# jesselasse/MARL-DMFB

Hardware: AMD Instinct MI355X
Metric: env-steps/sec (whole node), 10x10 DMFB 4-droplet fov9 (higher is better)
Workload: dtype int8 env state/obs + f64 rewards; fp32 Q-net; 1 GPU; DMFB 10x10, drop_num=4, fov=9, 4096 parallel envs per GPU (BASELINE configs[1]); parallelism=dp1: chips sharded per rank, one flat RCCL all-reduce per learn

## Files before the change

### __graft_entry__.py

```python
import os
import subprocess
import sys

ROOT = os.path.dirname(os.path.abspath(__file__))
if ROOT not in sys.path:
    sys.path.insert(0, ROOT)


def build():
    jobs = str(max(1, min(8, os.cpu_count() or 1)))
    env = dict(os.environ, PYTORCH_ROCM_ARCH='gfx950')
    subprocess.check_call(['make', '-C', os.path.join(ROOT, 'marl_dmfb_amd', 'csrc'), '-j', jobs, '-s'], env=env)
    subprocess.check_call(['make', '-C', os.path.join(ROOT, 'oracle'), '-s'], env=env)
    import marl_dmfb_amd
    from marl_dmfb_amd import _lib
    lib = _lib.dmfb_vec()
    for name in _lib.DMFB_VEC_SYMBOLS:
        getattr(lib, name)
    lib = _lib.meda_vec()
    for name in _lib.MEDA_VEC_SYMBOLS:
        getattr(lib, name)
    lib = _lib.crnn_ops()
    for name in ('crnn_conv9_forward', 'crnn_front9_forward', 'crnn_front19_forward', 'crnn_front_padded_cols', 'crnn_conv9_backward', 'crnn_conv19_backward', 'crnn_front9_forward_live', 'gru_seq_forward', 'gru_seq_backward', 'gru_seq_forward_packed', 'gru_seq_backward_packed'):
        getattr(lib, name)
    lib = _lib.crnn_fov()
    for name in _lib.SIGNATURES['crnn_fov']:
        getattr(lib, name)
    lib = _lib.rollout_ops()
    for name in ('rollout_select_actions', 'rollout_post_step', 'rollout_gru_head_select_stream', 'rollout_stream_step'):
        getattr(lib, name)
    lib = _lib.vdn_ops()
    for name in ('vdn_td_forward', 'vdn_td_backward', 'vdn_td_forward_packed', 'vdn_td_backward_packed', 'vdn_gather_units', 'vdn_clip_adam_step'):
        getattr(lib, name)
    lib = _lib.qmix_ops()
    for name in _lib.SIGNATURES['qmix_ops']:
        getattr(lib, name)
    lib = _lib.route_plan()
    for name in _lib.SIGNATURES['route_plan']:
        getattr(lib, name)


def smoke():
    import numpy as np
    import torch
    from marl_dmfb_amd.env.dmfb import VecDMFB
    from oracle.dmfb_oracle import DmfbOracle

    assert torch.cuda.is_available(), 'smoke() needs the GPU'
    cfg = dict(width=10, length=10, n_agents=4, fov=9)
    E, seed = 256, 1234
    env = VecDMFB(n_envs=E, seed=seed, device='cuda:0', **cfg)
    ora = DmfbOracle(n_envs=E, seed=seed, **cfg)
    env.reset()
    ora.reset()
    rng = np.random.default_rng(0)
    for t in range(50):
        a = rng.integers(0, 5, (E, 4)).astype(np.int32)
        obs, r, d, info = env.step(torch.as_tensor(a, device='cuda:0'), autoreset=True)
        ro, do, co, so = ora.step(a)
        term = do.all(axis=1)
        if term.any():
            ora.reset(mask=term.astype(np.uint8))
        assert np.array_equal(r.cpu().numpy().view(np.int64), ro.view(np.int64)), 'rewards differ at step %d' % t
        assert np.array_equal(d.cpu().numpy(), do), 'dones differ at step %d' % t
        assert np.array_equal(info['constraints'].cpu().numpy(), co)
# ... 26 lines not shown
```

### marl_dmfb_amd/_lib.py

```python
import ctypes as C
import os

_HERE = os.path.dirname(os.path.abspath(__file__))
LIB_DIR = os.path.join(_HERE, 'lib')
_CACHE = {}
_FILE = {'rollout_route': 'rollout_ops'}


class HipLibraryMissing(RuntimeError):
    pass


def load(name):
    if name in _CACHE:
        return _CACHE[name]
    stem = _FILE.get(name, name)
    path = os.path.join(LIB_DIR, 'lib%s%s.so' % (stem, os.environ.get('MARL_DMFB_VARIANT_' + stem.upper(), '')))
    if not os.path.exists(path):
        raise HipLibraryMissing(
            '%s not found: build the HIP extension first (python -c "import __graft_entry__ as g; g.build()" '
            'or make -C marl_dmfb_amd/csrc). There is no CPU fallback.' % path)
    import torch
    lib = C.CDLL(path)
    _CACHE[name] = lib
    return lib


class DmfbVecConfig(C.Structure):
    _fields_ = [('width', C.c_int32), ('length', C.c_int32), ('n_agents', C.c_int32), ('n_blocks', C.c_int32),
                ('fov', C.c_int32), ('stall', C.c_int32), ('b_degrade', C.c_int32), ('with_maps', C.c_int32),
                ('per_degrade', C.c_double), ('n_envs', C.c_int32), ('env_id0', C.c_uint32), ('seed', C.c_uint64),
                ('device', C.c_int32)]


class DmfbVecStepOut(C.Structure):
    _fields_ = [('d_rewards', C.c_void_p), ('d_dones', C.c_void_p), ('d_constraints', C.c_void_p),
                ('d_success', C.c_void_p), ('d_obs', C.c_void_p), ('d_team_reward', C.c_void_p),
                ('d_terminated', C.c_void_p), ('d_obs_terminal', C.c_void_p)]

# ... 130 lines not shown
        'rollout_select_actions': [vp, i32, i32, i32, vp, i32, u64, vp, vp, vp, vp, vp, i32, i32, vp],
        'rollout_gru_head_select': [vp, vp, vp, vp, vp, vp, vp, i32, i32, i32, i32, vp, i32, u64, vp, vp, vp, vp, vp, i32, i32, vp, vp],
        'rollout_gru_head_select_live': [vp, vp, vp, vp, vp, vp, vp, i32, i32, i32, i32, vp, i32, u64, vp, vp, vp, vp, vp, i32, i32, vp, vp,
                                         vp, vp],
        'rollout_compact_alive': [i32, vp, vp, vp, vp],
        'rollout_post_step': [i32, i32, i32, vp, vp, vp, vp, i32, vp, vp, vp, vp, vp, vp, vp, vp, vp, f32, f32, vp, vp, vp, i32, vp, vp,
                              vp],
        'rollout_gru_head_select_stream': [vp, vp, vp, vp, vp, vp, vp, i32, i32, i32, i32, vp, i32, u64, vp, vp, vp, vp, vp, i32, vp, vp,
                                           vp],
        'rollout_stream_step': [i32, i32, i32, i32, i32, i32, vp, vp, vp, vp, vp, vp, i32, vp, C.POINTER(RolloutStage),
                                C.POINTER(RolloutRing), i32, vp, vp, vp, f32, f32, vp, vp],
        'rollout_last_hip_error': ([], i32),
    },
    'rollout_route': {
        'rollout_route_select': [i32, i32, i32, i32, vp, vp, vp, i32, vp, vp, vp, vp, vp, vp],
        'rollout_last_hip_error': ([], i32),
    },
    'route_plan': {
        'route_plan_dmfb': [i32, i32, i32, i32, i32, vp, vp, vp, vp, vp, vp, vp, vp, vp, vp, vp],
        'route_plan_max_dim': ([], i32),
        'route_plan_lds_bytes': ([i32, i32, i32], i32),
        'route_plan_last_hip_error': ([], i32),
    },
    'vdn_ops': {
        'vdn_td_forward': [vp, vp, vp, vp, vp, vp, vp, i32, i32, i32, i32, i32, f32, vp, vp, vp, vp],
        'vdn_td_backward': [vp, vp, vp, vp, i32, i32, i32, i32, i32, vp, vp],
        'vdn_td_forward_packed': [vp, vp, vp, i32, vp, vp, vp, vp, vp, i32, i32, f32, vp, vp, vp, vp],
        'vdn_td_backward_packed': [vp, vp, vp, i32, vp, vp, i32, i32, vp, vp],
        'vdn_gather_units': [vp, i32, vp, i32, i32, i32, vp, vp],
        'vdn_clip_adam_step': [i32, C.POINTER(vp), C.POINTER(vp), C.POINTER(vp), C.POINTER(vp), C.POINTER(i64), f32, f64, f64, f64,
                               f64, f64, f64, vp, vp, vp, vp],
        'vdn_last_hip_error': ([], i32),
    },
    'qmix_ops': {
        'qmix_mix_td_forward': [vp, vp, vp, vp, vp, vp, vp, i32, i32, i32, i32, i32, vp, i32, i32, vp, i32, i32, i32, i32,
                                C.POINTER(QmixMixer), C.POINTER(QmixMixer), f32, vp, vp, vp, vp],
        'qmix_mix_td_backward': [vp, vp, vp, vp, i32, i32, i32, i32, i32, vp, i32, i32, i32, i32, C.POINTER(QmixMixer), vp, vp, vp,
                                 vp, vp, vp],
        'qmix_last_hip_error': ([], i32),
    },
}

DMFB_VEC_SYMBOLS = list(SIGNATURES['dmfb_vec'])
MEDA_VEC_SYMBOLS = list(SIGNATURES['meda_vec'])

ENV_ERRORS = {
    'dmfb_vec': {
        -1: (ValueError, 'bad argument'),
        -2: (RuntimeError, 'Fov is too large'),
        -3: (TypeError, 'Too many droplets for DMFB'),
        -4: (AssertionError, 'width >= 5 and length >= 5'),
        -5: (AssertionError, 'n_agents > 0'),
        -6: (NotImplementedError, 'configuration outside the build limits (include/dmfb_vec.h)'),
        -7: (TypeError, 'action is illegal'),
        -8: (RuntimeError, 'env was created without health/usage/degrade maps (pass with_maps=True)'),
    },
    'meda_vec': {
        -1: (ValueError, 'bad argument'),
        -3: (RuntimeError, 'Too many droplets in the MEDA array'),
        -4: (AssertionError, 'w > 0 and l > 0'),
        -5: (AssertionError, 'n_agents > 0'),
        -6: (NotImplementedError, 'configuration outside the build limits (include/meda_vec.h)'),
        -8: (RuntimeError, 'env was created without health/usage/degrade maps (pass with_maps=True)'),
    },
    'route_plan': {
        -1: (ValueError, 'bad argument'),
# ... 57 lines not shown

def dmfb_vec():
    return _library('dmfb_vec')


def meda_vec():
    return _library('meda_vec')


def crnn_ops():
    return _library('crnn_ops')


def crnn_fov():
    return _library('crnn_fov')


def rollout_ops():
    return _library('rollout_ops')


def rollout_route():
    return _library('rollout_route')


def route_plan():
    return _library('route_plan')


def vdn_ops():
    return _library('vdn_ops')


def qmix_ops():
    return _library('qmix_ops')
```

### marl_dmfb_amd/csrc/crnn_ops.hip

```cpp
#include <hip/hip_runtime.h>

#include <cstdint>
#include <cstdio>
#include <cstdlib>

#include "../../include/crnn_ops.h"

#define HIP_ABI_TAG "crnn_ops"
#define HIP_ABI_ERR CRNN_ERR_HIP
#include "hip_abi.h"
#include "crnn_mfma.h"
#include "crnn_mfma19.h"
#include "crnn_bwd19.h"

namespace {

constexpr int kBlock = 512;
constexpr int kA1Stride = 52;
constexpr int kDz1Unit = 108;

constexpr int kLdsBudget = 158 * 1024;

template <int OD> struct GeoB {
    static constexpr int DZ2 = 28;
// ... 337 lines not shown
            const int pair = i / 9, tap = i - pair * 9, c2 = pair / OD, c1 = pair - c2 * OD;
            const int unit = c2 * (OD / 2) + (c1 >> 1), comp = 2 * tap + (c1 & 1);
            if (unit < G::NA) off[cnt++] = unit * 18 + comp;
            else
                for (int sl = 0; sl < G::XSLICES && sl < 8; ++sl) off[cnt++] = (G::NA + sl * G::NB + (unit - G::NA)) * 18 + comp;
        } else if (i < n2 + nb) {
            off[cnt++] = kBlock * 18 + (i - n2);
        } else if (i < n2 + nb + n1) {
            const int jx = i - n2 - nb, c1 = jx / 27, r = jx - c1 * 27, ky = r % 3;
            const int item = (c1 >> 1) * 9 + r / 3;
            for (int sl = 0; sl < G::RS3; ++sl) off[cnt++] = kBlock * 18 + OD + (sl * G::ITEMS3 + item) * 6 + (c1 & 1) * 3 + ky;
        } else {
            off[cnt++] = kBlock * 18 + OD + kBlock * 6 + (i - n2 - nb - n1);
        }
        for (int k = 0; k < cnt; ++k) {
            float a0 = 0.0f, a1 = 0.0f;
            int b = ty;
            for (; b + kRedY < n_part; b += 2 * kRedY) { a0 += part[(size_t)b * G::PART + off[k]]; a1 += part[(size_t)(b + kRedY) * G::PART + off[k]]; }
            if (b < n_part) a0 += part[(size_t)b * G::PART + off[k]];
            acc += a0 + a1;
        }
    }
    s_sum[ty][tx] = acc;
    __syncthreads();
    if (ty == 0 && i < n2 + nb + n1 + nb) {
        float t = 0.0f;
#pragma unroll
        for (int k = 0; k < kRedY; ++k) t += s_sum[k][tx];
        grads[i] = t;
    }
}

constexpr int kMlpBlock = 256, kMlpOut = 10, kMlpMaxIn = 18, kMlpMaxParts = 256;
__global__ __launch_bounds__(kMlpBlock) void k_mlp_bwd(const int8_t *__restrict__ obs, long obs_stride, int dir_off,
                                                       const int8_t *__restrict__ onehot, int n_actions, long rows,
                                                       const float *__restrict__ x, long x_stride, const float *__restrict__ g, long g_stride,
                                                       int col0, float *__restrict__ part) {
    __shared__ float s_red[kMlpBlock / 64][kMlpOut * (kMlpMaxIn + 1)];
    float acc[kMlpOut][kMlpMaxIn + 1];
#pragma unroll
    for (int o = 0; o < kMlpOut; ++o)
#pragma unroll
        for (int k = 0; k <= kMlpMaxIn; ++k) acc[o][k] = 0.0f;
    for (long r = (long)blockIdx.x * kMlpBlock + threadIdx.x; r < rows; r += (long)gridDim.x * kMlpBlock) {
        float v[kMlpMaxIn];
        v[0] = (float)obs[r * obs_stride + dir_off];
        v[1] = (float)obs[r * obs_stride + dir_off + 1];
#pragma unroll
        for (int k = 0; k < kMlpMaxIn - 2; ++k) v[2 + k] = k < n_actions ? (float)onehot[r * n_actions + k] : 0.0f;
#pragma unroll
        for (int o = 0; o < kMlpOut; ++o) {
            const float gz = x[r * x_stride + col0 + o] > 0.0f ? g[r * g_stride + col0 + o] : 0.0f;
#pragma unroll
            for (int k = 0; k < kMlpMaxIn; ++k) acc[o][k] = fmaf(gz, v[k], acc[o][k]);
            acc[o][kMlpMaxIn] += gz;
        }
    }
    const int lane = threadIdx.x & 63, wave = threadIdx.x >> 6;
#pragma unroll
    for (int o = 0; o < kMlpOut; ++o)
#pragma unroll
        for (int k = 0; k <= kMlpMaxIn; ++k) {
            float t = acc[o][k];
            for (int d = 32; d > 0; d >>= 1) t += __shfl_xor(t, d);
            if (lane == 0) s_red[wave][o * (kMlpMaxIn + 1) + k] = t;
        }
    __syncthreads();
    for (int i = threadIdx.x; i < kMlpOut * (kMlpMaxIn + 1); i += kMlpBlock) {
        float t = 0.0f;
#pragma unroll
        for (int w = 0; w < kMlpBlock / 64; ++w) t += s_red[w][i];
        part[(size_t)blockIdx.x * kMlpOut * (kMlpMaxIn + 1) + i] = t;
    }
}
__global__ __launch_bounds__(256) void k_mlp_bwd_reduce(const float *__restrict__ part, int n_part, int nin, float *__restrict__ dw, float *__restrict__ db) {
    const int i = threadIdx.x;
    if (i >= kMlpOut * nin + kMlpOut) return;
    const int o = i < kMlpOut * nin ? i / nin : i - kMlpOut * nin, k = i < kMlpOut * nin ? i - o * nin : kMlpMaxIn;
    float t = 0.0f;
    for (int b = 0; b < n_part; ++b) t += part[(size_t)b * kMlpOut * (kMlpMaxIn + 1) + o * (kMlpMaxIn + 1) + k];
    if (i < kMlpOut * nin) dw[i] = t;
    else db[o] = t;
}

struct LiveRows { const int32_t *chips; const int32_t *n; int rows_per_chip; };

template <int OD, int RBV>
int launch_rb(const int8_t *obs, long obs_stride, long rows, const float *w1, const float *b1, const float *w2, const float *b2,
              float *out, long out_stride, int out_cols, const int8_t *onehot, int n_actions, const float *mlp_w, const float *mlp_b, hipStream_t s,
              LiveRows live = LiveRows{nullptr, nullptr, 1}) {
    using GM = crnn_mfma::GeoM<OD, RBV>;
    const size_t lds = GM::LDS_FLOATS * sizeof(float);
    static LdsLimit lds_limit;
    if (const int rc = lds_limit.raise((const void *)crnn_mfma::k_conv9_mfma<OD, RBV>, lds)) return rc;
    const long n_blocks = (rows + GM::RB - 1) / GM::RB;
    const long resident = 256L * (long)((size_t)160 * 1024 / lds);
    const int grid = (int)(n_blocks < resident ? n_blocks : resident);
    LAUNCH((crnn_mfma::k_conv9_mfma<OD, RBV>), dim3(grid), dim3(crnn_mfma::kBlockM), lds, s, obs, obs_stride, rows, w1, b1, w2, b2,
           out, out_stride, out_cols, onehot, n_actions, mlp_w, mlp_b, live.chips, live.n, live.rows_per_chip);
    return CRNN_OK;
}

template <int OD>
int launch(const int8_t *obs, long obs_stride, long rows, const float *w1, const float *b1, const float *w2, const float *b2,
           float *out, long out_stride, int out_cols, const int8_t *onehot, int n_actions, const float *mlp_w, const float *mlp_b, hipStream_t s,
           LiveRows live = LiveRows{nullptr, nullptr, 1}) {
    return launch_rb<OD, 0>(obs, obs_stride, rows, w1, b1, w2, b2, out, out_stride, out_cols, onehot, n_actions, mlp_w, mlp_b, s, live);
}

template <int OD>
int launch19(const int8_t *obs, long obs_stride, long rows, const float *w1, const float *b1, const float *w3, const float *b3,
             float *out, long out_stride, int out_cols, const int8_t *onehot, int n_actions, const float *mlp_w, const float *mlp_b, hipStream_t s) {
    using GM = crnn_mfma19::Geo<OD>;
    const size_t lds = GM::LDS_FLOATS * sizeof(float);
    static LdsLimit lds_limit;
// ... 90 lines not shown
    const bool vec = d_mlp_w != nullptr;
    const int n_feat = od * 25 + (vec ? 10 : 0);
    if (!d_obs || !d_w1 || !d_b1 || !d_w3 || !d_b3 || !d_out || rows < 0 || obs_stride < 3 * 19 * 19 + (vec ? 2 : 0) ||
        out_stride < n_feat || n_actions < 0 || n_actions > 16 || (vec && !d_mlp_b))
        return CRNN_ERR_BAD_ARG;
    if (od != 24 && od != 32) return CRNN_ERR_UNSUPPORTED;
    if (out_cols != 0 && (out_cols < n_feat || out_cols > crnn_front_padded_cols(od) || out_cols > out_stride)) return CRNN_ERR_BAD_ARG;
    if (rows == 0) return CRNN_OK;
    if (od == 24) return launch19<24>(d_obs, obs_stride, rows, d_w1, d_b1, d_w3, d_b3, d_out, out_stride, out_cols, d_onehot, n_actions, d_mlp_w, d_mlp_b, (hipStream_t)stream);
    return launch19<32>(d_obs, obs_stride, rows, d_w1, d_b1, d_w3, d_b3, d_out, out_stride, out_cols, d_onehot, n_actions, d_mlp_w, d_mlp_b, (hipStream_t)stream);
}

int crnn_conv9_backward_parts(int od) { return od == 24 ? GeoB<24>::PART : od == 32 ? GeoB<32>::PART : CRNN_ERR_UNSUPPORTED; }

int crnn_conv9_backward(const int8_t *d_obs, int64_t obs_stride, int64_t rows, const float *d_out, int64_t out_stride,
                        const float *d_grad_out, int64_t grad_stride, const float *d_w1, const float *d_b1, const float *d_w2,
                        int od, float *d_part, int n_part, float *d_grads, void *stream) {
    if (!d_obs || !d_out || !d_grad_out || !d_w1 || !d_b1 || !d_w2 || !d_part || !d_grads || rows <= 0 || n_part < 1 || n_part > 256)
        return CRNN_ERR_BAD_ARG;
    if (od == 24) return launch_bwd<24>(d_obs, obs_stride, rows, d_out, out_stride, d_grad_out, grad_stride, d_w2, d_part, n_part, d_grads, d_w1, d_b1, (hipStream_t)stream);
    if (od == 32) return launch_bwd<32>(d_obs, obs_stride, rows, d_out, out_stride, d_grad_out, grad_stride, d_w2, d_part, n_part, d_grads, d_w1, d_b1, (hipStream_t)stream);
    return CRNN_ERR_UNSUPPORTED;
}

int crnn_mlp_backward_parts(void) { return kMlpMaxParts * kMlpOut * (kMlpMaxIn + 1); }

int crnn_mlp_backward(const int8_t *d_obs, int64_t obs_stride, int dir_offset, const int8_t *d_onehot, int n_actions, int64_t rows,
                      const float *d_out, int64_t out_stride, const float *d_grad_out, int64_t grad_stride, int col0, float *d_part,
                      float *d_grad_w, float *d_grad_b, void *stream) {
    if (!d_obs || !d_onehot || !d_out || !d_grad_out || !d_part || !d_grad_w || !d_grad_b || rows <= 0 || n_actions < 0 ||
        n_actions > kMlpMaxIn - 2 || dir_offset < 0 || obs_stride < dir_offset + 2 || col0 < 0 || out_stride < col0 + kMlpOut ||
        grad_stride < col0 + kMlpOut)
        return CRNN_ERR_BAD_ARG;
    const long want = (rows + kMlpBlock - 1) / kMlpBlock;
    const int grid = (int)(want < kMlpMaxParts ? want : kMlpMaxParts);
    HIP_TRY(launch_status([&] {
        hipLaunchKernelGGL(k_mlp_bwd, dim3(grid), dim3(kMlpBlock), 0, (hipStream_t)stream, d_obs, (long)obs_stride, dir_offset, d_onehot, n_actions,
                           (long)rows, d_out, (long)out_stride, d_grad_out, (long)grad_stride, col0, d_part);
        hipLaunchKernelGGL(k_mlp_bwd_reduce, dim3(1), dim3(256), 0, (hipStream_t)stream, d_part, grid, 2 + n_actions, d_grad_w, d_grad_b);
    }));
    return CRNN_OK;
}

int crnn_conv19_backward_parts(int od) { return od == 24 ? crnn_bwd19::GeoB19<24>::PART : od == 32 ? crnn_bwd19::GeoB19<32>::PART : CRNN_ERR_UNSUPPORTED; }

int crnn_conv19_backward(const int8_t *d_obs, int64_t obs_stride, int64_t rows, const float *d_out, int64_t out_stride,
                         const float *d_grad_out, int64_t grad_stride, const float *d_w1, const float *d_b1, const float *d_w3,
                         const float *d_b3, int od, float *d_part, int n_part, float *d_grads, void *stream) {
    if (!d_obs || !d_out || !d_grad_out || !d_w1 || !d_b1 || !d_w3 || !d_b3 || !d_part || !d_grads || rows <= 0 || n_part < 1 ||
        n_part > 256 || obs_stride < 3 * 19 * 19 || out_stride < od * 25 || grad_stride < od * 25)
        return CRNN_ERR_BAD_ARG;
    if (od == 24) return launch_bwd19<24>(d_obs, obs_stride, rows, d_out, out_stride, d_grad_out, grad_stride, d_w1, d_b1, d_w3, d_b3, d_part, n_part, d_grads, (hipStream_t)stream);
    if (od == 32) return launch_bwd19<32>(d_obs, obs_stride, rows, d_out, out_stride, d_grad_out, grad_stride, d_w1, d_b1, d_w3, d_b3, d_part, n_part, d_grads, (hipStream_t)stream);
    return CRNN_ERR_UNSUPPORTED;
}

int crnn_last_hip_error(void) { return g_last_hip; }

}
```

### marl_dmfb_amd/csrc/vdn_ops.hip

```cpp
#include <hip/hip_runtime.h>

#include <cstdint>

#include "../../include/vdn_ops.h"

#define HIP_ABI_TAG "vdn_ops"
#define HIP_ABI_ERR VDN_ERR_HIP
#include "hip_abi.h"

namespace {

__global__ __launch_bounds__(256) void k_td_forward(const float *__restrict__ qe, const float *__restrict__ qt, const int8_t *__restrict__ u,
                                                    const float *__restrict__ r, const int8_t *__restrict__ avail,
                                                    const uint8_t *__restrict__ term, const uint8_t *__restrict__ padded, int B, int T,
                                                    int Tl, int n, int A, float gamma, float *__restrict__ mtd, float *__restrict__ maskf,
                                                    int32_t *__restrict__ bad) {
    const int idx = blockIdx.x * blockDim.x + threadIdx.x;
    if (idx >= B * T) return;
    const int b = idx / T, t = idx - b * T;
    const size_t ep = (size_t)b * Tl + t;
    const size_t q0 = ((size_t)t * B + b) * n * A;
    float qe_tot = 0.0f, qt_tot = 0.0f;
    bool ok = true;
    for (int i = 0; i < n; ++i) {
        int a_taken = (int)u[ep * n + i];
        if ((unsigned)a_taken >= (unsigned)A) { ok = false; a_taken = 0; }
        qe_tot = qe_tot + qe[q0 + (size_t)i * A + a_taken];
        float m = -3.4e38f;
        for (int a = 0; a < A; ++a) {
            const float v = avail[(ep * n + i) * A + a] == 0 ? -9999999.0f : qt[q0 + (size_t)i * A + a];
            m = v > m ? v : m;
        }
        qt_tot = qt_tot + m;
    }
    const float not_term = 1.0f - (term[ep] ? 1.0f : 0.0f);
    const float target = r[ep] + (gamma * qt_tot) * not_term;
    const float mk = 1.0f - (padded[ep] ? 1.0f : 0.0f);
// ... 39 lines not shown
        }
        qt_tot = qt_tot + m;
    }
    const float not_term = 1.0f - (term[ep] ? 1.0f : 0.0f);
    const float target = r[ep] + (gamma * qt_tot) * not_term;
    const float mk = 1.0f - (padded[ep] ? 1.0f : 0.0f);
    mtd[j] = ok ? mk * (target - qe_tot) : __builtin_nanf("");
    maskf[j] = mk;
    if (!ok && bad) atomicAdd(bad, 1);
}

__global__ __launch_bounds__(256) void k_td_backward_packed(const float *__restrict__ mtd, const float *__restrict__ maskf, const int32_t *__restrict__ units,
                                                            const int8_t *__restrict__ u, const float *__restrict__ g, long rows, int n, int A,
                                                            float *__restrict__ gq) {
    const long row = (long)blockIdx.x * blockDim.x + threadIdx.x;
    if (row >= rows) return;
    const int i = (int)(row % n);
    const long j = row / n;
    const float d = -((2.0f * mtd[j]) * maskf[j]) * g[0];
    const int a_taken = (int)u[(size_t)units[j] * n + i];
    const bool bad_a = (unsigned)a_taken >= (unsigned)A;
    for (int a = 0; a < A; ++a) gq[row * A + a] = (bad_a || a == a_taken) ? d : 0.0f;
}

template <typename V>
__global__ __launch_bounds__(256) void k_gather_units(const V *__restrict__ src, int unit_v, const int32_t *__restrict__ units, int U, int shift,
                                                      int zero_below, V *__restrict__ dst) {
    const long idx = (long)blockIdx.x * blockDim.x + threadIdx.x;
    if (idx >= (long)U * unit_v) return;
    const int j = (int)(idx / unit_v), k = (int)(idx - (long)j * unit_v);
    dst[idx] = j < zero_below ? (V)0 : src[((size_t)units[j] + shift) * unit_v + k];
}

}

namespace {

struct TensorList {
    float *p[VDN_MAX_TENSORS];
    float *g[VDN_MAX_TENSORS];
    float *m[VDN_MAX_TENSORS];
    float *v[VDN_MAX_TENSORS];
    long off[VDN_MAX_TENSORS + 1];
    int n;
};

__device__ __forceinline__ void locate(const TensorList &tl, long i, int &k) {
    while (i >= tl.off[k + 1]) ++k;
}

__global__ __launch_bounds__(256) void k_sqnorm_partials(TensorList tl, float *__restrict__ partials, const float *__restrict__ grad_div) {
    __shared__ float s_w[4];
    const long total = tl.off[tl.n];
    const long per = (total + gridDim.x - 1) / gridDim.x;
    const long lo = (long)blockIdx.x * per, hi = min(total, lo + per);
    float acc = 0.0f;
    int k = 0;
    for (long i = lo + threadIdx.x; i < hi; i += 256) {
        locate(tl, i, k);
        float g = tl.g[k][i - tl.off[k]];
        if (grad_div) g = g / grad_div[0];
        acc = fmaf(g, g, acc);
    }
    for (int o = 32; o > 0; o >>= 1) acc += __shfl_xor(acc, o);
    if ((threadIdx.x & 63) == 0) s_w[threadIdx.x >> 6] = acc;
    __syncthreads();
// ... 111 lines not shown
           d_bad_actions);
    return VDN_OK;
}

int vdn_td_backward_packed(const float *d_mtd, const float *d_mask, const int32_t *d_units, int32_t n_units, const int8_t *d_u,
                           const float *d_grad_num, int32_t n_agents, int32_t n_actions, float *d_grad_q, void *stream) {
    if (!d_mtd || !d_mask || !d_units || !d_u || !d_grad_num || !d_grad_q || n_units < 0 || n_agents < 1 || n_actions < 1 || n_actions > 127)
        return VDN_ERR_BAD_ARG;
    if (n_units == 0) return VDN_OK;
    const long rows = (long)n_units * n_agents;
    LAUNCH(k_td_backward_packed, dim3((unsigned)((rows + 255) / 256)), dim3(256), 0, (hipStream_t)stream, d_mtd, d_mask, d_units,
           d_u, d_grad_num, rows, n_agents, n_actions, d_grad_q);
    return VDN_OK;
}

int vdn_gather_units(const void *d_src, int32_t unit_bytes, const int32_t *d_units, int32_t n_units, int32_t unit_shift,
                     int32_t zero_below, void *d_dst, void *stream) {
    if (!d_src || !d_units || !d_dst || unit_bytes < 1 || n_units < 0 || zero_below < 0) return VDN_ERR_BAD_ARG;
    if (n_units == 0) return VDN_OK;
    HIP_TRY(launch_status([&] {
        const bool dw = unit_bytes % 4 == 0 && ((size_t)d_src | (size_t)d_dst) % 4 == 0;
        const int uv = dw ? unit_bytes / 4 : unit_bytes;
        const long total = (long)n_units * uv;
        if (dw)
            hipLaunchKernelGGL((k_gather_units<uint32_t>), dim3((unsigned)((total + 255) / 256)), dim3(256), 0, (hipStream_t)stream,
                               (const uint32_t *)d_src, uv, d_units, n_units, unit_shift, zero_below, (uint32_t *)d_dst);
        else
            hipLaunchKernelGGL((k_gather_units<uint8_t>), dim3((unsigned)((total + 255) / 256)), dim3(256), 0, (hipStream_t)stream,
                               (const uint8_t *)d_src, uv, d_units, n_units, unit_shift, zero_below, (uint8_t *)d_dst);
    }));
    return VDN_OK;
}

int vdn_last_hip_error(void) { return g_last_hip; }

}
```

### marl_dmfb_amd/network/base_net.py

```python
import os

import torch
import torch.nn as nn
import torch.nn.functional as f


_CONV_PLAN = {5: [(True, 1)], 7: [(True, 1), (False, 1)], 9: [(True, 1), (False, 1)], 11: [(True, 1), (False, 1)],
              13: [(True, 1), (False, 1)], 19: [(True, 2), (False, 1), (False, 1)]}


class _ConvGemm(torch.autograd.Function):

    @staticmethod
    def forward(ctx, cols, weight2d, bias):
        ctx.save_for_backward(cols, weight2d)
        return torch.addmm(bias, cols, weight2d.t())

    @staticmethod
    def backward(ctx, g):
        cols, w = ctx.saved_tensors
        g = g.contiguous()
        gcols = g @ w if ctx.needs_input_grad[0] else None
        M, K = cols.shape
        C = g.shape[1]
# ... 289 lines not shown
        hs, gates, h0, w_hh = ctx.saved_tensors
        lib = _GRUSeqHip._lib()
        T, R, H = hs.shape
        grad_out = grad_out.contiguous()
        h0c, w = h0.contiguous(), w_hh.contiguous()
        d_ig = torch.empty((T, R, 3 * H), dtype=torch.float32, device=hs.device)
        d_hg = torch.empty_like(d_ig)
        d_h0 = torch.empty_like(h0c)
        bias_part = torch.empty((lib.gru_seq_row_blocks(R), 6 * H), dtype=torch.float32, device=hs.device)
        lib.gru_seq_backward(grad_out.data_ptr(), gates.data_ptr(), hs.data_ptr(), h0c.data_ptr(),
                             w.data_ptr(), T, R, H, d_ig.data_ptr(), d_hg.data_ptr(), d_h0.data_ptr(),
                             bias_part.data_ptr(), torch.cuda.current_stream(hs.device).cuda_stream)
        d_w_hh = torch.matmul(d_hg[0].t(), h0c)
        if T > 1:
            d_w_hh = d_w_hh + _wgrad_splitk(d_hg[1:].reshape((T - 1) * R, 3 * H), hs[:-1].reshape((T - 1) * R, H))
        d_b = bias_part.sum(0)
        return d_ig, d_h0, d_w_hh, d_b[:3 * H], d_b[3 * H:]


class _GRUSeqHipPacked(torch.autograd.Function):

    @staticmethod
    def _steps(step_rows):
        import ctypes as C
        return (C.c_int32 * len(step_rows))(*[int(v) for v in step_rows])

    @staticmethod
    def run_forward(igates, h0, w_hh, b_ih, b_hh, step_rows, save):
        lib = _GRUSeqHip._lib()
        Vp, G = igates.shape
        H, T, R, V = G // 3, len(step_rows), h0.shape[0], int(sum(step_rows))
        igates, h0, w_hh = igates.contiguous(), h0.contiguous(), w_hh.contiguous()
        hs = torch.empty((Vp, H), dtype=torch.float32, device=igates.device)
        hs[V:].zero_()
        gates = torch.empty((Vp, 4 * H), dtype=torch.float32, device=igates.device) if save else None
        lib.gru_seq_forward_packed(igates.data_ptr(), h0.data_ptr(), w_hh.data_ptr(), b_ih.data_ptr(),
                                   b_hh.data_ptr(), T, R, H, _GRUSeqHipPacked._steps(step_rows), hs.data_ptr(),
                                   gates.data_ptr() if save else None,
                                   torch.cuda.current_stream(igates.device).cuda_stream)
        return hs, gates

    @staticmethod
    def forward(ctx, igates, h0, w_hh, b_ih, b_hh, step_rows):
        hs, gates = _GRUSeqHipPacked.run_forward(igates.detach(), h0.detach(), w_hh.detach(), b_ih.detach(), b_hh.detach(), step_rows, True)
        ctx.save_for_backward(hs, gates, h0, w_hh)
        ctx.step_rows = list(step_rows)
        return hs

    @staticmethod
    def backward(ctx, grad_out):
        hs, gates, h0, w_hh = ctx.saved_tensors
        lib = _GRUSeqHip._lib()
        step_rows = ctx.step_rows
        Vp, H = hs.shape
        T, R, V = len(step_rows), h0.shape[0], int(sum(step_rows))
        grad_out = grad_out.contiguous()
        h0c, w = h0.contiguous(), w_hh.contiguous()
        d_ig = torch.empty((Vp, 3 * H), dtype=torch.float32, device=hs.device)
        d_hg = torch.empty_like(d_ig)
        h_prev = torch.empty((Vp, H), dtype=torch.float32, device=hs.device)
        for t in (d_ig, d_hg, h_prev):
            t[V:].zero_()
        d_h0 = torch.zeros_like(h0c)
        bias_part = torch.empty((lib.gru_seq_row_blocks(R), 6 * H), dtype=torch.float32, device=hs.device)
        lib.gru_seq_backward_packed(grad_out.data_ptr(), gates.data_ptr(), hs.data_ptr(), h0c.data_ptr(),
                                    w.data_ptr(), T, R, H, _GRUSeqHipPacked._steps(step_rows), d_ig.data_ptr(),
                                    d_hg.data_ptr(), d_h0.data_ptr(), bias_part.data_ptr(), h_prev.data_ptr(),
                                    torch.cuda.current_stream(hs.device).cuda_stream)
        d_w_hh = _wgrad_splitk(d_hg, h_prev)
        d_b = bias_part.sum(0)
        return d_ig, d_h0, d_w_hh, d_b[:3 * H], d_b[3 * H:], None


class _GRUSeqPairPacked(torch.autograd.Function):

    @staticmethod
    def forward(ctx, ig_a, w_hh_a, b_ih_a, b_hh_a, ig_b, w_hh_b, b_ih_b, b_hh_b, step_rows, R):
        lib = _GRUSeqHip._lib()
        Vp, G = ig_a.shape
        Hd, T, V = G // 3, len(step_rows), int(sum(step_rows))
        save = any(ctx.needs_input_grad[:4])
        ta = [t.detach().contiguous() for t in (ig_a, w_hh_a, b_ih_a, b_hh_a)]
        tb = [t.detach().contiguous() for t in (ig_b, w_hh_b, b_ih_b, b_hh_b)]
        hs_a = torch.empty((Vp, Hd), dtype=torch.float32, device=ig_a.device)
        hs_b = torch.empty((Vp, Hd), dtype=torch.float32, device=ig_a.device)
        hs_a[V:].zero_()
        hs_b[V:].zero_()
        gates = torch.empty((Vp, 4 * Hd), dtype=torch.float32, device=ig_a.device) if save else None
        lib.gru_seq_forward_packed_pair(ta[0].data_ptr(), None, ta[1].data_ptr(), ta[2].data_ptr(), ta[3].data_ptr(),
                                        hs_a.data_ptr(), gates.data_ptr() if save else None,
                                        tb[0].data_ptr(), None, tb[1].data_ptr(), tb[2].data_ptr(), tb[3].data_ptr(),
                                        hs_b.data_ptr(), None, T, R, Hd, _GRUSeqHipPacked._steps(step_rows),
                                        torch.cuda.current_stream(ig_a.device).cuda_stream)
        if save:
            h0 = torch.zeros((R, Hd), dtype=torch.float32, device=ig_a.device)
            ctx.save_for_backward(hs_a, gates, h0, ta[1])
            ctx.step_rows = list(step_rows)
        ctx.mark_non_differentiable(hs_b)
        return hs_a, hs_b

    @staticmethod
    def backward(ctx, grad_a, _grad_b):
        d_ig, _d_h0, d_w_hh, d_b_ih, d_b_hh, _ = _GRUSeqHipPacked.backward(ctx, grad_a)
        return d_ig, d_w_hh, d_b_ih, d_b_hh, None, None, None, None, None, None


def gru_sequence(igates, h0, w_hh, b_ih, b_hh, impl='hip'):
    if impl == 'hip' and h0.shape[-1] == 128 and igates.dtype == torch.float32:
        if torch.is_grad_enabled() and any(t.requires_grad for t in (igates, h0, w_hh, b_ih, b_hh)):
            return _GRUSeqHip.apply(igates, h0, w_hh, b_ih, b_hh)
        return _GRUSeqHip.run_forward(igates, h0, w_hh, b_ih, b_hh, False)[0]
    return _GRUSeq.apply(igates, h0, w_hh, b_ih, b_hh)


def conv_str(fov, id=3, od=32):
    stack, shared = [], None
    for from_image, stride in _CONV_PLAN[fov]:
        if from_image:
            stack.append(nn.Conv2d(id, od, kernel_size=3, stride=stride))
        else:
            if shared is None:
                shared = nn.Conv2d(od, od, kernel_size=3, stride=stride)
            stack.append(shared)
    return stack


class CRNN(nn.Module):
    def __init__(self, args):
        super().__init__()
# ... 251 lines not shown
```

### marl_dmfb_amd/policy/vdn.py

```python
import os

import torch

from ..network.base_net import CRNN, RNN
from ..network.vdn_net import VDNNet


def _t(x, device, dtype):
    if not isinstance(x, torch.Tensor):
        x = torch.as_tensor(x)
    return x.to(device=device, dtype=dtype)


def _episode_slots(t):
    inner = 1
    for k in range(t.dim() - 1, 0, -1):
        if t.stride(k) != inner and t.shape[k] != 1:
            return None
        inner *= t.shape[k]
    per_step = inner // t.shape[1]
    if t.shape[0] == 1:
        return t.shape[1]
    if per_step == 0 or t.stride(0) % per_step or t.stride(0) // per_step < t.shape[1]:
        return None
# ... 278 lines not shown
                'u_onehot': torch.int8, 'o_next': torch.int8}
        if any(not (isinstance(buffers.get(k), torch.Tensor) and buffers[k].dtype == dt and buffers[k].is_contiguous()) for k, dt in want.items()):
            return False
        probe = o.view(-1, o.shape[-1])[:1]
        with torch.no_grad():
            return bool(hasattr(net, '_hip_conv_ok') and net._hip_conv_ok(probe) and net._hip_geometry() in (5, 7, 9, 19)
                        and hasattr(net, '_hip_train_ok'))

    @staticmethod
    def pack_units(idx, lens, t_ring):
        import numpy as np
        idx, lens = np.asarray(idx, np.int64), np.asarray(lens, np.int64)
        counts = (lens[None, :] > np.arange(int(lens[0]))[:, None]).sum(1)
        units = np.concatenate([idx[:c] * t_ring + t for t, c in enumerate(counts)]).astype(np.int32)
        return counts, units

    def learn_packed(self, buffers, idx, lens, train_step, plan=None):
        import numpy as np
        dev, n, A = self.device, self.n_agents, self.n_actions
        B, T_ring, O = len(idx), buffers['o'].shape[1], buffers['o'].shape[-1]
        if plan is None:
            counts, units_np = self.pack_units(idx, lens, T_ring)
            units = torch.from_numpy(units_np).to(dev, non_blocking=True)
        else:
            counts, units = plan
        U = int(units.shape[0])
        V = U * n
        pad = PACK_ROWS if V >= 32768 else 64
        Vp = -(-V // pad) * pad
        from .. import _lib
        lib = _lib.checked('vdn_ops')
        stream = torch.cuda.current_stream(dev).cuda_stream

        def packed(src, shift=0, zero_below=0):
            row = src.shape[-1]
            out = torch.empty((Vp, row), dtype=src.dtype, device=dev)
            out[V:].zero_()
            lib.vdn_gather_units(src.data_ptr(), n * row * src.element_size(), units.data_ptr(), U, shift,
                                 zero_below, out.data_ptr(), stream)
            return out
        obs_e, obs_t, oh_t = packed(buffers['o']), packed(buffers['o_next']), packed(buffers['u_onehot'])
        oh_e = packed(buffers['u_onehot'], shift=-1, zero_below=B)
        x_e = self._features(self.eval_rnn, obs_e, oh_e)
        with torch.no_grad():
            x_t = self._features(self.target_rnn, obs_t, oh_t)
        step_rows = [int(c) * n for c in counts]
        if os.environ.get('MARL_DMFB_GRU_PAIR', '1') != '0' and hasattr(self.eval_rnn, 'recurrent_seq_packed_pair'):
            q_e, q_t = self.eval_rnn.recurrent_seq_packed_pair(self.eval_rnn, x_e, self.target_rnn, x_t, step_rows, B * n)
        else:
            q_e = self.eval_rnn.recurrent_seq_packed(x_e, step_rows, B * n)
            with torch.no_grad():
                q_t = self.target_rnn.recurrent_seq_packed(x_t, step_rows, B * n)
        if self._td_bad is None:
            self._td_bad = torch.zeros(1, dtype=torch.int32, device=dev)
        num, mask_sum = _TDLossPacked.apply(q_e, q_t, units, U, buffers['u'], buffers['r'], buffers['avail_u_next'],
                                            buffers['terminated'], buffers['padded'], n, A, self.args.gamma, self._td_bad)
        return self._backward_and_step(num, mask_sum, train_step)

    def check_td_inputs(self):
        if self._td_bad is not None:
            bad = int(self._td_bad.item())
            if bad:
                self._td_bad.zero_()
                raise RuntimeError('%s.learn: %d (episode, step) slots with an action outside [0, %d)' % (type(self).__name__, bad, self.n_actions))

    def _fused_step(self, grad_div=None):
        a = self.args
        params = [p for p in self.eval_parameters if p.grad is not None]
        ok = (self.device.type == 'cuda' and a.optimizer == 'ADAM' and getattr(a, 'fused_clip_adam', True) and 0 < len(params) <= 32
              and all(p.dtype == torch.float32 and p.grad.dtype == torch.float32 and p.is_contiguous() and p.grad.is_contiguous()
                      for p in params))
        if getattr(self, '_fused_choice', None) is None:
            self._fused_choice = ok
        elif self._fused_choice != ok:
            raise RuntimeError('VDN: the clip + Adam step changed from %s to %s between two learns (gradient layout / dtype / set of '
# ... 131 lines not shown
```

Measured before the change: 7.455 million env-steps/s.

## Batch learn-step gathers into one kernel and retile MLP backward reduction

The four per-buffer unit gathers and their tail-zero fills in packed VDN learning become one multi-source gather kernel, which also zero-fills padding rows. The small MLP weight-gradient kernel now stages tiles of rows in shared memory, with one thread per (output, input) weight, and its partial reduction is spread over many small blocks. Redundant zero fills are skipped when there is no padding, and the zero initial hidden state is cached instead of allocated each call. These trim launch overhead and register pressure in the learner tail; the learner is a modest share of env-steps throughput.

```diff
diff --git a/__graft_entry__.py b/__graft_entry__.py
--- a/__graft_entry__.py
+++ b/__graft_entry__.py
@@ -31,6 +31,9 @@
         getattr(lib, name)
     lib = _lib.vdn_ops()
     for name in ('vdn_td_forward', 'vdn_td_backward', 'vdn_td_forward_packed', 'vdn_td_backward_packed', 'vdn_gather_units', 'vdn_clip_adam_step'):
+        getattr(lib, name)
+    lib = _lib.vdn_pack()
+    for name in _lib.SIGNATURES['vdn_pack']:
         getattr(lib, name)
     lib = _lib.qmix_ops()
     for name in _lib.SIGNATURES['qmix_ops']:
diff --git a/include/vdn_pack.h b/include/vdn_pack.h
--- /dev/null
+++ b/include/vdn_pack.h
@@ -0,0 +1,18 @@
+#ifndef VDN_PACK_H
+#define VDN_PACK_H
+
+#include <stdint.h>
+
+#ifdef __cplusplus
+extern "C" {
+#endif
+
+#define VDN_MAX_GATHER 4
+int vdn_gather_units_multi(int32_t n_src, const void *const *d_src, const int32_t *unit_bytes, const int32_t *unit_shift,
+                           const int32_t *zero_below, void *const *d_dst, const int64_t *dst_bytes, const int32_t *d_units,
+                           int32_t n_units, void *stream);
+
+#ifdef __cplusplus
+}
+#endif
+#endif
diff --git a/marl_dmfb_amd/_lib.py b/marl_dmfb_amd/_lib.py
--- a/marl_dmfb_amd/_lib.py
+++ b/marl_dmfb_amd/_lib.py
@@ -4,7 +4,7 @@
 _HERE = os.path.dirname(os.path.abspath(__file__))
 LIB_DIR = os.path.join(_HERE, 'lib')
 _CACHE = {}
-_FILE = {'rollout_route': 'rollout_ops'}
+_FILE = {'rollout_route': 'rollout_ops', 'vdn_pack': 'vdn_ops'}
 
 
 class HipLibraryMissing(RuntimeError):
@@ -201,6 +201,10 @@
                                f64, f64, f64, vp, vp, vp, vp],
         'vdn_last_hip_error': ([], i32),
     },
+    'vdn_pack': {
+        'vdn_gather_units_multi': [i32, C.POINTER(vp), C.POINTER(i32), C.POINTER(i32), C.POINTER(i32), C.POINTER(vp), C.POINTER(i64), vp,
+                                   i32, vp],
+    },
     'qmix_ops': {
         'qmix_mix_td_forward': [vp, vp, vp, vp, vp, vp, vp, i32, i32, i32, i32, i32, vp, i32, i32, vp, i32, i32, i32, i32,
                                 C.POINTER(QmixMixer), C.POINTER(QmixMixer), f32, vp, vp, vp, vp],
@@ -324,5 +328,9 @@
     return _library('vdn_ops')
 
 
+def vdn_pack():
+    return _library('vdn_pack')
+
+
 def qmix_ops():
     return _library('qmix_ops')
diff --git a/marl_dmfb_amd/csrc/crnn_ops.hip b/marl_dmfb_amd/csrc/crnn_ops.hip
--- a/marl_dmfb_amd/csrc/crnn_ops.hip
+++ b/marl_dmfb_amd/csrc/crnn_ops.hip
@@ -393,55 +393,59 @@
 }
 
 constexpr int kMlpBlock = 256, kMlpOut = 10, kMlpMaxIn = 18, kMlpMaxParts = 256;
+constexpr int kMlpTile = 384, kMlpVS = kMlpMaxIn + 1, kMlpMinRows = 64;
+constexpr int kMlpLd = (kMlpTile * kMlpOut + kMlpBlock - 1) / kMlpBlock;
 __global__ __launch_bounds__(kMlpBlock) void k_mlp_bwd(const int8_t *__restrict__ obs, long obs_stride, int dir_off,
-                                                       const int8_t *__restrict__ onehot, int n_actions, long rows,
+                                                       const int8_t *__restrict__ onehot, int n_actions, long rows, long rows_per_wg,
                                                        const float *__restrict__ x, long x_stride, const float *__restrict__ g, long g_stride,
                                                        int col0, float *__restrict__ part) {
-    __shared__ float s_red[kMlpBlock / 64][kMlpOut * (kMlpMaxIn + 1)];
-    float acc[kMlpOut][kMlpMaxIn + 1];
-#pragma unroll
-    for (int o = 0; o < kMlpOut; ++o)
-#pragma unroll
-        for (int k = 0; k <= kMlpMaxIn; ++k) acc[o][k] = 0.0f;
-    for (long r = (long)blockIdx.x * kMlpBlock + threadIdx.x; r < rows; r += (long)gridDim.x * kMlpBlock) {
-        float v[kMlpMaxIn];
-        v[0] = (float)obs[r * obs_stride + dir_off];
-        v[1] = (float)obs[r * obs_stride + dir_off + 1];
-#pragma unroll
-        for (int k = 0; k < kMlpMaxIn - 2; ++k) v[2 + k] = k < n_actions ? (float)onehot[r * n_actions + k] : 0.0f;
-#pragma unroll
-        for (int o = 0; o < kMlpOut; ++o) {
-            const float gz = x[r * x_stride + col0 + o] > 0.0f ? g[r * g_stride + col0 + o] : 0.0f;
-#pragma unroll
-            for (int k = 0; k < kMlpMaxIn; ++k) acc[o][k] = fmaf(gz, v[k], acc[o][k]);
-            acc[o][kMlpMaxIn] += gz;
-        }
-    }
-    const int lane = threadIdx.x & 63, wave = threadIdx.x >> 6;
-#pragma unroll
-    for (int o = 0; o < kMlpOut; ++o)
-#pragma unroll
-        for (int k = 0; k <= kMlpMaxIn; ++k) {
-            float t = acc[o][k];
-            for (int d = 32; d > 0; d >>= 1) t += __shfl_xor(t, d);
-            if (lane == 0) s_red[wave][o * (kMlpMaxIn + 1) + k] = t;
-        }
-    __syncthreads();
-    for (int i = threadIdx.x; i < kMlpOut * (kMlpMaxIn + 1); i += kMlpBlock) {
-        float t = 0.0f;
-#pragma unroll
-        for (int w = 0; w < kMlpBlock / 64; ++w) t += s_red[w][i];
-        part[(size_t)blockIdx.x * kMlpOut * (kMlpMaxIn + 1) + i] = t;
-    }
-}
-__global__ __launch_bounds__(256) void k_mlp_bwd_reduce(const float *__restrict__ part, int n_part, int nin, float *__restrict__ dw, float *__restrict__ db) {
-    const int i = threadIdx.x;
-    if (i >= kMlpOut * nin + kMlpOut) return;
-    const int o = i < kMlpOut * nin ? i / nin : i - kMlpOut * nin, k = i < kMlpOut * nin ? i - o * nin : kMlpMaxIn;
+    __shared__ float s_gz[kMlpTile * kMlpOut];
+    __shared__ float s_v[kMlpTile * kMlpVS];
+    const int tid = threadIdx.x, nin = 2 + n_actions, nk = nin + 1;
+    const int o = tid / nk, k = tid - o * nk;
+    const bool owner = tid < kMlpOut * nk;
+    const long lo = (long)blockIdx.x * rows_per_wg, hi = min(rows, lo + rows_per_wg);
+    float acc = 0.0f;
+    for (long r0 = lo; r0 < hi; r0 += kMlpTile) {
+        const int n = (int)min((long)kMlpTile, hi - r0);
+        float xv[kMlpLd], gv[kMlpLd];
+#pragma unroll
+        for (int j = 0; j < kMlpLd; ++j) {
+            const int i = tid + j * kMlpBlock, r = i / kMlpOut, c = i - r * kMlpOut;
+            const bool in = i < n * kMlpOut;
+            xv[j] = in ? x[(r0 + r) * x_stride + col0 + c] : 0.0f;
+            gv[j] = in ? g[(r0 + r) * g_stride + col0 + c] : 0.0f;
+        }
+        for (int i = tid; i < n * 2; i += kMlpBlock)
+            s_v[(i >> 1) * kMlpVS + (i & 1)] = (float)obs[(r0 + (i >> 1)) * obs_stride + dir_off + (i & 1)];
+        for (int i = tid; i < n * n_actions; i += kMlpBlock) {
+            const int r = i / n_actions;
+            s_v[r * kMlpVS + 2 + (i - r * n_actions)] = (float)onehot[r0 * n_actions + i];
+        }
+        for (int i = tid; i < n; i += kMlpBlock) s_v[i * kMlpVS + nin] = 1.0f;
+#pragma unroll
+        for (int j = 0; j < kMlpLd; ++j) {
+            const int i = tid + j * kMlpBlock;
+            if (i < n * kMlpOut) s_gz[i] = xv[j] > 0.0f ? gv[j] : 0.0f;
+        }
+        __syncthreads();
+        if (owner) {
+#pragma unroll 8
+            for (int r = 0; r < n; ++r) acc = fmaf(s_gz[r * kMlpOut + o], s_v[r * kMlpVS + k], acc);
+        }
+        __syncthreads();
+    }
+    if (owner) part[(size_t)tid * gridDim.x + blockIdx.x] = acc;
+}
+__global__ __launch_bounds__(64) void k_mlp_bwd_reduce(const float *__restrict__ part, int n_part, int nin, float *__restrict__ dw, float *__restrict__ db) {
+    const int i = blockIdx.x, o = i / (nin + 1), k = i - o * (nin + 1);
     float t = 0.0f;
-    for (int b = 0; b < n_part; ++b) t += part[(size_t)b * kMlpOut * (kMlpMaxIn + 1) + o * (kMlpMaxIn + 1) + k];
-    if (i < kMlpOut * nin) dw[i] = t;
-    else db[o] = t;
+    for (int b = threadIdx.x; b < n_part; b += 64) t += part[(size_t)i * n_part + b];
+    for (int d = 32; d > 0; d >>= 1) t += __shfl_xor(t, d);
+    if (threadIdx.x == 0) {
+        if (k < nin) dw[o * nin + k] = t;
+        else db[o] = t;
+    }
 }
 
 struct LiveRows { const int32_t *chips; const int32_t *n; int rows_per_chip; };
@@ -598,12 +602,14 @@
         n_actions > kMlpMaxIn - 2 || dir_offset < 0 || obs_stride < dir_offset + 2 || col0 < 0 || out_stride < col0 + kMlpOut ||
         grad_stride < col0 + kMlpOut)
         return CRNN_ERR_BAD_ARG;
-    const long want = (rows + kMlpBlock - 1) / kMlpBlock;
+    const long want = (rows + kMlpMinRows - 1) / kMlpMinRows;
     const int grid = (int)(want < kMlpMaxParts ? want : kMlpMaxParts);
+    const long rows_per_wg = (rows + grid - 1) / grid;
     HIP_TRY(launch_status([&] {
         hipLaunchKernelGGL(k_mlp_bwd, dim3(grid), dim3(kMlpBlock), 0, (hipStream_t)stream, d_obs, (long)obs_stride, dir_offset, d_onehot, n_actions,
-                           (long)rows, d_out, (long)out_stride, d_grad_out, (long)grad_stride, col0, d_part);
-        hipLaunchKernelGGL(k_mlp_bwd_reduce, dim3(1), dim3(256), 0, (hipStream_t)stream, d_part, grid, 2 + n_actions, d_grad_w, d_grad_b);
+                           (long)rows, rows_per_wg, d_out, (long)out_stride, d_grad_out, (long)grad_stride, col0, d_part);
+        hipLaunchKernelGGL(k_mlp_bwd_reduce, dim3(kMlpOut * (3 + n_actions)), dim3(64), 0, (hipStream_t)stream, d_part, grid, 2 + n_actions,
+                           d_grad_w, d_grad_b);
     }));
     return CRNN_OK;
 }
diff --git a/marl_dmfb_amd/csrc/vdn_ops.hip b/marl_dmfb_amd/csrc/vdn_ops.hip
--- a/marl_dmfb_amd/csrc/vdn_ops.hip
+++ b/marl_dmfb_amd/csrc/vdn_ops.hip
@@ -3,6 +3,7 @@
 #include <cstdint>
 
 #include "../../include/vdn_ops.h"
+#include "../../include/vdn_pack.h"
 
 #define HIP_ABI_TAG "vdn_ops"
 #define HIP_ABI_ERR VDN_ERR_HIP
@@ -108,6 +109,42 @@
     dst[idx] = j < zero_below ? (V)0 : src[((size_t)units[j] + shift) * unit_v + k];
 }
 
+template <typename V>
+struct GatherList {
+    const V *src[VDN_MAX_GATHER];
+    V *dst[VDN_MAX_GATHER];
+    long total_v[VDN_MAX_GATHER];
+    int unit_v[VDN_MAX_GATHER], shift[VDN_MAX_GATHER], zero_below[VDN_MAX_GATHER];
+};
+template <typename V>
+__global__ __launch_bounds__(256) void k_gather_units_multi(GatherList<V> gl, const int32_t *__restrict__ units, int U) {
+    const int s = blockIdx.y, unit_v = gl.unit_v[s];
+    const long idx = (long)blockIdx.x * blockDim.x + threadIdx.x;
+    if (idx >= gl.total_v[s]) return;
+    const long j = idx / unit_v;
+    const int k = (int)(idx - j * unit_v);
+    gl.dst[s][idx] = (j >= U || j < gl.zero_below[s]) ? (V)0 : gl.src[s][((size_t)units[j] + gl.shift[s]) * unit_v + k];
+}
+
+template <typename V>
+void launch_gather_multi(int n_src, const void *const *src, const int32_t *unit_bytes, const int32_t *shift, const int32_t *zero_below,
+                         void *const *dst, const int64_t *dst_bytes, const int32_t *units, int U, hipStream_t stream) {
+    GatherList<V> gl;
+    long most = 0;
+    for (int s = 0; s < VDN_MAX_GATHER; ++s) {
+        const bool on = s < n_src;
+        gl.src[s] = on ? (const V *)src[s] : nullptr;
+        gl.dst[s] = on ? (V *)dst[s] : nullptr;
+        gl.total_v[s] = on ? (long)(dst_bytes[s] / (int64_t)sizeof(V)) : 0;
+        gl.unit_v[s] = on ? unit_bytes[s] / (int)sizeof(V) : 1;
+        gl.shift[s] = on ? shift[s] : 0;
+        gl.zero_below[s] = on ? zero_below[s] : 0;
+        most = gl.total_v[s] > most ? gl.total_v[s] : most;
+    }
+    if (most == 0) return;
+    hipLaunchKernelGGL((k_gather_units_multi<V>), dim3((unsigned)((most + 255) / 256), n_src), dim3(256), 0, stream, gl, units, U);
+}
+
 }
 
 namespace {
@@ -285,6 +322,27 @@
     return VDN_OK;
 }
 
+int vdn_gather_units_multi(int32_t n_src, const void *const *d_src, const int32_t *unit_bytes, const int32_t *unit_shift,
+                           const int32_t *zero_below, void *const *d_dst, const int64_t *dst_bytes, const int32_t *d_units,
+                           int32_t n_units, void *stream) {
+    if (n_src < 1 || n_src > VDN_MAX_GATHER || !d_src || !unit_bytes || !unit_shift || !zero_below || !d_dst || !dst_bytes || !d_units ||
+        n_units < 0)
+        return VDN_ERR_BAD_ARG;
+    bool dw = true;
+    for (int s = 0; s < n_src; ++s) {
+        if (!d_src[s] || !d_dst[s] || unit_bytes[s] < 1 || zero_below[s] < 0 || dst_bytes[s] < (int64_t)n_units * unit_bytes[s])
+            return VDN_ERR_BAD_ARG;
+        dw = dw && unit_bytes[s] % 4 == 0 && dst_bytes[s] % 4 == 0 && ((size_t)d_src[s] | (size_t)d_dst[s]) % 4 == 0;
+    }
+    HIP_TRY(launch_status([&] {
+        if (dw)
+            launch_gather_multi<uint32_t>(n_src, d_src, unit_bytes, unit_shift, zero_below, d_dst, dst_bytes, d_units, n_units, (hipStream_t)stream);
+        else
+            launch_gather_multi<uint8_t>(n_src, d_src, unit_bytes, unit_shift, zero_below, d_dst, dst_bytes, d_units, n_units, (hipStream_t)stream);
+    }));
+    return VDN_OK;
+}
+
 int vdn_last_hip_error(void) { return g_last_hip; }
 
 }
diff --git a/marl_dmfb_amd/network/base_net.py b/marl_dmfb_amd/network/base_net.py
--- a/marl_dmfb_amd/network/base_net.py
+++ b/marl_dmfb_amd/network/base_net.py
@@ -345,7 +345,8 @@
         H, T, R, V = G // 3, len(step_rows), h0.shape[0], int(sum(step_rows))
         igates, h0, w_hh = igates.contiguous(), h0.contiguous(), w_hh.contiguous()
         hs = torch.empty((Vp, H), dtype=torch.float32, device=igates.device)
-        hs[V:].zero_()
+        if V < Vp:
+            hs[V:].zero_()
         gates = torch.empty((Vp, 4 * H), dtype=torch.float32, device=igates.device) if save else None
         lib.gru_seq_forward_packed(igates.data_ptr(), h0.data_ptr(), w_hh.data_ptr(), b_ih.data_ptr(),
                                    b_hh.data_ptr(), T, R, H, _GRUSeqHipPacked._steps(step_rows), hs.data_ptr(),
@@ -372,8 +373,9 @@
         d_ig = torch.empty((Vp, 3 * H), dtype=torch.float32, device=hs.device)
         d_hg = torch.empty_like(d_ig)
         h_prev = torch.empty((Vp, H), dtype=torch.float32, device=hs.device)
-        for t in (d_ig, d_hg, h_prev):
-            t[V:].zero_()
+        if V < Vp:
+            for t in (d_ig, d_hg, h_prev):
+                t[V:].zero_()
         d_h0 = torch.zeros_like(h0c)
         bias_part = torch.empty((lib.gru_seq_row_blocks(R), 6 * H), dtype=torch.float32, device=hs.device)
         lib.gru_seq_backward_packed(grad_out.data_ptr(), gates.data_ptr(), hs.data_ptr(), h0c.data_ptr(),
@@ -385,6 +387,16 @@
         return d_ig, d_h0, d_w_hh, d_b[:3 * H], d_b[3 * H:], None
 
 
+_ZERO_H0 = {}
+
+
+def _zero_h0(R, H, device):
+    key = (R, H, str(device))
+    if key not in _ZERO_H0:
+        _ZERO_H0[key] = torch.zeros((R, H), dtype=torch.float32, device=device)
+    return _ZERO_H0[key]
+
+
 class _GRUSeqPairPacked(torch.autograd.Function):
 
     @staticmethod
@@ -397,8 +409,9 @@
         tb = [t.detach().contiguous() for t in (ig_b, w_hh_b, b_ih_b, b_hh_b)]
         hs_a = torch.empty((Vp, Hd), dtype=torch.float32, device=ig_a.device)
         hs_b = torch.empty((Vp, Hd), dtype=torch.float32, device=ig_a.device)
-        hs_a[V:].zero_()
-        hs_b[V:].zero_()
+        if V < Vp:
+            hs_a[V:].zero_()
+            hs_b[V:].zero_()
         gates = torch.empty((Vp, 4 * Hd), dtype=torch.float32, device=ig_a.device) if save else None
         lib.gru_seq_forward_packed_pair(ta[0].data_ptr(), None, ta[1].data_ptr(), ta[2].data_ptr(), ta[3].data_ptr(),
                                         hs_a.data_ptr(), gates.data_ptr() if save else None,
@@ -406,8 +419,7 @@
                                         hs_b.data_ptr(), None, T, R, Hd, _GRUSeqHipPacked._steps(step_rows),
                                         torch.cuda.current_stream(ig_a.device).cuda_stream)
         if save:
-            h0 = torch.zeros((R, Hd), dtype=torch.float32, device=ig_a.device)
-            ctx.save_for_backward(hs_a, gates, h0, ta[1])
+            ctx.save_for_backward(hs_a, gates, _zero_h0(R, Hd, ig_a.device), ta[1])
             ctx.step_rows = list(step_rows)
         ctx.mark_non_differentiable(hs_b)
         return hs_a, hs_b
diff --git a/marl_dmfb_amd/policy/vdn.py b/marl_dmfb_amd/policy/vdn.py
--- a/marl_dmfb_amd/policy/vdn.py
+++ b/marl_dmfb_amd/policy/vdn.py
@@ -334,15 +334,23 @@
         lib = _lib.checked('vdn_ops')
         stream = torch.cuda.current_stream(dev).cuda_stream
 
-        def packed(src, shift=0, zero_below=0):
-            row = src.shape[-1]
-            out = torch.empty((Vp, row), dtype=src.dtype, device=dev)
-            out[V:].zero_()
-            lib.vdn_gather_units(src.data_ptr(), n * row * src.element_size(), units.data_ptr(), U, shift,
-                                 zero_below, out.data_ptr(), stream)
-            return out
-        obs_e, obs_t, oh_t = packed(buffers['o']), packed(buffers['o_next']), packed(buffers['u_onehot'])
-        oh_e = packed(buffers['u_onehot'], shift=-1, zero_below=B)
+        sources = ((buffers['o'], 0, 0), (buffers['o_next'], 0, 0), (buffers['u_onehot'], 0, 0), (buffers['u_onehot'], -1, B))
+        outs = [torch.empty((Vp, src.shape[-1]), dtype=src.dtype, device=dev) for src, _, _ in sources]
+        if os.environ.get('MARL_DMFB_LEARN_TAIL', '1') != '0':
+            import ctypes as C
+            k = len(sources)
+            _lib.checked('vdn_pack').vdn_gather_units_multi(
+                k, (C.c_void_p * k)(*[src.data_ptr() for src, _, _ in sources]),
+                (C.c_int32 * k)(*[n * src.shape[-1] * src.element_size() for src, _, _ in sources]),
+                (C.c_int32 * k)(*[shift for _, shift, _ in sources]), (C.c_int32 * k)(*[zb for _, _, zb in sources]),
+                (C.c_void_p * k)(*[out.data_ptr() for out in outs]), (C.c_int64 * k)(*[out.numel() * out.element_size() for out in outs]),
+                units.data_ptr(), U, stream)
+        else:
+            for (src, shift, zero_below), out in zip(sources, outs):
+                out[V:].zero_()
+                lib.vdn_gather_units(src.data_ptr(), n * src.shape[-1] * src.element_size(), units.data_ptr(), U, shift,
+                                     zero_below, out.data_ptr(), stream)
+        obs_e, obs_t, oh_t, oh_e = outs
         x_e = self._features(self.eval_rnn, obs_e, oh_e)
         with torch.no_grad():
             x_t = self._features(self.target_rnn, obs_t, oh_t)
```

After: 7.619 million env-steps/s (median of 6 runs). 2.2% higher.
